# kubernetes-sigs/scheduler-plugins

Hardware: AMD Instinct MI355X
Metric: pod_x_node_filter_score_evals_per_sec (higher is better)
Workload: dtype f32+f64

## Files before the change

### include/spx.h

```cpp
#ifndef SPX_H
#define SPX_H

#include <stdint.h>

#ifdef __cplusplus
extern "C" {
#endif


#define SPX_OK 0
#define SPX_ERR_ARG (-1)
#define SPX_ERR_HIP (-2)
#define SPX_ERR_STATE (-3)
#define SPX_ERR_NOGPU (-4)

#define SPX_PLUGIN_ALLOCATABLE 0
#define SPX_PLUGIN_TLP 1
#define SPX_PLUGIN_LVRB 2
#define SPX_PLUGIN_NRT 3
#define SPX_PLUGIN_NETOVERHEAD 4
#define SPX_PLUGIN_CAPACITY 5
#define SPX_PLUGIN_TOPOSORT 6
#define SPX_PLUGIN_LROC 7
#define SPX_PLUGIN_PEAKS 8
// ... 751 lines not shown
#define SPX_OPT_PEAKS_POD_CLASSES 8
#define SPX_OPT_NRT_LN_LIST_PERMILLE 9
#define SPX_OPT_COMMIT_COOP 10
#define SPX_OPT_NRT_RANK_FILTER 11
#define SPX_OPT_ROW_WORKGROUP 12
#define SPX_OPT_TLP_AMB_TABLE 13
#define SPX_OPT_NRT_PACKED_SCORE 14
#define SPX_OPT_NET_ALLOC_FUSED 15
#define SPX_OPT_NRT_RANK_NARROW 16
#define SPX_OPT_PEAKS_ESTIMATE 17
#define SPX_OPT_NRT_FUSED 18
#define SPX_OPT_NRT_WIDE 19
#define SPX_OPT_ALLOC_TABLE_KEEP 20
#define SPX_OPT_TLP_POD_CLASSES 21
#define SPX_OPT_TLP_CHUNK_SCHED 22
#define SPX_NUM_OPTIONS 23
int spx_set_option(spx_engine* e, int option, int64_t value);
int spx_get_option(const spx_engine* e, int option, int64_t* value);

int spx_nrt_pod_classes(const spx_engine* e, int64_t* n_unique, int64_t* n_copies);
int spx_peaks_pod_classes(const spx_engine* e, int64_t* n_unique, int64_t* n_copies);

int spx_tlp_pod_classes(const spx_engine* e, int64_t* rows_evaluated, int64_t* rows_copied);
int spx_tlp_form(const spx_engine* e);
int spx_tlp_fetch_order(spx_engine* e, int32_t* rows);

int spx_sysched_pod_classes(const spx_engine* e, int64_t* n_unique, int64_t* n_copies);

int spx_load_trimaran(spx_engine* e, const spx_node_objects* nodes, const spx_resource_classes* rc, const spx_pod_objects* pods, const spx_metrics_objects* metrics, const spx_assigned_objects* assigned);
int spx_load_trimaran_pods(spx_engine* e, const spx_pod_objects* pods);
int spx_load_nrt(spx_engine* e, const spx_node_objects* nodes, const spx_nrt_objects* nrt, const spx_resource_classes* rc, const spx_pod_objects* pods, const spx_nrt_params* params);
int spx_last_load_nrt_ms(const spx_engine* e, double* ms6);
int spx_load_network(spx_engine* e, const spx_node_objects* nodes, const spx_pod_objects* pods, const spx_appgroup_objects* appgroups, const spx_nettopo_objects* nettopo);
int spx_load_quota(spx_engine* e, const spx_pod_objects* pods, const spx_resource_classes* rc, const spx_quota_objects* quota);
int spx_load_sysched(spx_engine* e, const spx_sysched_objects* o);
typedef struct spx_profile_objects {
  const spx_node_objects* nodes;
  const spx_resource_classes* rc;
  const spx_pod_objects* pods;
  const spx_metrics_objects* metrics;
// ... 133 lines not shown
```

### scheduler-plugins_amd/csrc/kernels_tlp_order.hip

```cpp
#include <hip/hip_runtime.h>

#include "spx_internal.h"

namespace spx {
namespace {

constexpr int kBlock = 1024;
constexpr int kSlots = 2 * kBlock;
constexpr uint32_t kEmpty = 0xffffffffu;

__device__ __forceinline__ uint32_t order_bin(int64_t v, int32_t amb_size) {
  return (v >= 0 && v < static_cast<int64_t>(amb_size)) ? static_cast<uint32_t>(v) : static_cast<uint32_t>(amb_size);
}

__device__ __forceinline__ void block_count(uint32_t* skey, uint32_t* scnt, bool live, uint32_t bin, uint32_t* slot, uint32_t* rank) {
  for (int s = threadIdx.x; s < kSlots; s += kBlock) skey[s] = kEmpty, scnt[s] = 0u;
  __syncthreads();
  *slot = 0u, *rank = 0u;
  if (live) {
    uint32_t s = (bin * 2654435761u) >> 21;
    for (;;) {
      const uint32_t prev = atomicCAS(skey + s, kEmpty, bin);
      if (prev == kEmpty || prev == bin) break;
      s = (s + 1u) & (kSlots - 1);
// ... 18 lines not shown
__device__ __forceinline__ uint32_t block_sum(uint32_t v, uint32_t* wsum) {
#pragma unroll
  for (int m = 32; m >= 1; m >>= 1) v += static_cast<uint32_t>(__shfl_xor(static_cast<int>(v), m));
  if ((threadIdx.x & 63) == 0) wsum[threadIdx.x >> 6] = v;
  __syncthreads();
  uint32_t total = 0;
#pragma unroll
  for (int w = 0; w < kBlock / 64; ++w) total += wsum[w];
  __syncthreads();
  return total;
}

__global__ __launch_bounds__(kBlock) void k_tlp_order_totals(const uint32_t* hist, int n_bins, uint32_t* totals) {
  __shared__ uint32_t wsum[kBlock / 64];
  const int b = blockIdx.x * kBlock + threadIdx.x;
  const uint32_t total = block_sum(b < n_bins ? hist[b] : 0u, wsum);
  if (threadIdx.x == 0) totals[blockIdx.x] = total;
}

__global__ __launch_bounds__(kBlock) void k_tlp_order_scan(uint32_t* hist, int n_bins, const uint32_t* totals, uint32_t* other_start, uint32_t* evaluated) {
  __shared__ uint32_t wsum[kBlock / 64];
  const int t = threadIdx.x, lane = t & 63, wave = t >> 6;
  uint32_t mine = 0;
  for (int i = t; i < static_cast<int>(blockIdx.x); i += kBlock) mine += totals[i];
  const uint32_t carry = block_sum(mine, wsum);
  const int b = blockIdx.x * kBlock + t;
  const uint32_t c = b < n_bins ? hist[b] : 0u;
  uint32_t x = c;
#pragma unroll
  for (int d = 1; d < 64; d <<= 1) {
    const uint32_t y = static_cast<uint32_t>(__shfl_up(static_cast<int>(x), d));
    if (lane >= d) x += y;
  }
  if (lane == 63) wsum[wave] = x;
  __syncthreads();
  uint32_t before = 0;
#pragma unroll
  for (int w = 0; w < kBlock / 64; ++w) before += w < wave ? wsum[w] : 0u;
  __syncthreads();
  const uint32_t o = carry + before + x - c;
  uint32_t ev = 0;
  if (b < n_bins) {
    hist[b] = o;
    if (b == n_bins - 1) *other_start = o;
    else if (c > 0u) ev = 1u + ((o + c - 1u) >> 6) - (o >> 6);
  }
  ev = block_sum(ev, wsum);
  if (t == 0 && ev != 0u) atomicAdd(evaluated, ev);
}

__global__ __launch_bounds__(kBlock) void k_tlp_order_scatter(const int64_t* pod, int64_t n, int32_t amb_size, uint32_t* cursor, int32_t* order) {
  __shared__ uint32_t skey[kSlots], scnt[kSlots];
  const int64_t r = static_cast<int64_t>(blockIdx.x) * kBlock + threadIdx.x;
  const bool live = r < n;
  uint32_t slot, rank;
  block_count(skey, scnt, live, live ? order_bin(pod[r], amb_size) : 0u, &slot, &rank);
  for (int s = threadIdx.x; s < kSlots; s += kBlock)
    if (skey[s] != kEmpty) scnt[s] = atomicAdd(cursor + skey[s], scnt[s]);
  __syncthreads();
  if (live) {
    const uint64_t pos = static_cast<uint64_t>(scnt[slot]) + rank;
    if (pos < static_cast<uint64_t>(n)) order[pos] = static_cast<int32_t>(r);
  }
}

__global__ __launch_bounds__(256) void k_tlp_order_count_key(const int64_t* pod, int64_t n, int32_t amb_size, const int32_t* order, const uint32_t* other_start,
                                                             uint32_t* evaluated, uint32_t* keys, int64_t n_chunks) {
  const int64_t p = static_cast<int64_t>(blockIdx.x) * blockDim.x + threadIdx.x;
  const uint32_t last = static_cast<uint32_t>(n - 1);
  bool ev = false, outside = false;
  if (p < n) {
    const int64_t v = pod[min(static_cast<uint32_t>(order[p]), last)];
    ev = (p & 63) == 0 || v != pod[min(static_cast<uint32_t>(order[p - 1]), last)];
    outside = order_bin(v, amb_size) == static_cast<uint32_t>(amb_size);
  }
  const unsigned long long m = __ballot(ev), mo = __ballot(ev && p >= static_cast<int64_t>(*other_start)), out = __ballot(outside);
  if ((threadIdx.x & 63) == 0) {
// ... 46 lines not shown
      for (int w = 0; w < kBlock / 64; ++w) add += wcnt[w][t], wcnt[w][t] = 0u;
      base[t] += add;
    }
    __syncthreads();
  }
}

__global__ __launch_bounds__(256) void k_tlp_order_move(int64_t n, const int32_t* sorted, const uint32_t* dest, int64_t n_chunks, int32_t* order) {
  const int64_t p = static_cast<int64_t>(blockIdx.x) * blockDim.x + threadIdx.x;
  if (p >= n) return;
  int64_t chunk = p >> 6;
  if (chunk < n_chunks) chunk = min(static_cast<int64_t>(dest[chunk]), n_chunks - 1);
  order[chunk * 64 + (p & 63)] = sorted[p];
}

}

static size_t scan_blocks(int32_t amb_size) { return (static_cast<size_t>(amb_size) + 1 + kBlock - 1) / kBlock; }
size_t tlp_order_scratch_words(int32_t amb_size, int64_t n_rows) {
  return static_cast<size_t>(amb_size) + 3 + scan_blocks(amb_size) + 2 * static_cast<size_t>(n_rows / 64) + static_cast<size_t>(n_rows);
}
size_t tlp_order_evaluated_word(int32_t amb_size) { return static_cast<size_t>(amb_size) + 2; }

void launch_tlp_order(const int64_t* pod_milli, int64_t n_rows, int32_t amb_size, bool chunk_sched, int32_t* order, uint32_t* scratch, hipStream_t s) {
  const int n_bins = amb_size + 1;
  const unsigned blocks = static_cast<unsigned>((n_rows + kBlock - 1) / kBlock), rows256 = static_cast<unsigned>((n_rows + 255) / 256);
  const unsigned sblocks = static_cast<unsigned>(scan_blocks(amb_size));
  const int64_t n_chunks = n_rows / 64;
  uint32_t* other_start = scratch + n_bins;
  uint32_t* evaluated = other_start + 1;
  uint32_t* totals = evaluated + 1;
  uint32_t* keys = totals + sblocks;
  uint32_t* dest = keys + n_chunks;
  const bool sched = chunk_sched && n_chunks > 1;
  int32_t* sorted = sched ? reinterpret_cast<int32_t*>(dest + n_chunks) : order;
  (void)hipMemsetAsync(scratch, 0, (static_cast<size_t>(n_bins) + 2) * sizeof(uint32_t), s);
  hipLaunchKernelGGL(k_tlp_order_hist, dim3(blocks), dim3(kBlock), 0, s, pod_milli, n_rows, amb_size, scratch);
  hipLaunchKernelGGL(k_tlp_order_totals, dim3(sblocks), dim3(kBlock), 0, s, scratch, n_bins, totals);
  hipLaunchKernelGGL(k_tlp_order_scan, dim3(sblocks), dim3(kBlock), 0, s, scratch, n_bins, totals, other_start, evaluated);
  hipLaunchKernelGGL(k_tlp_order_scatter, dim3(blocks), dim3(kBlock), 0, s, pod_milli, n_rows, amb_size, scratch, sorted);
  hipLaunchKernelGGL(k_tlp_order_count_key, dim3(rows256), dim3(256), 0, s, pod_milli, n_rows, amb_size, sorted, other_start, evaluated, keys, n_chunks);
  if (!sched) return;
  hipLaunchKernelGGL(k_tlp_order_sched, dim3(1), dim3(kBlock), 0, s, keys, n_chunks, dest);
  hipLaunchKernelGGL(k_tlp_order_move, dim3(rows256), dim3(256), 0, s, n_rows, sorted, dest, n_chunks, order);
}

}
```

### scheduler-plugins_amd/csrc/spx_engine.h

```cpp
#pragma once

#include <hip/hip_runtime.h>

#include <algorithm>
#include <chrono>
#include <cmath>
#include <cstdio>
#include <cstdlib>
#include <cstring>
#include <limits>
#include <string>
#include <unordered_map>
#include <vector>

#include <atomic>
#include <mutex>
#include <thread>

#include "spx_internal.h"
#include "../host/lroc_form.hpp"
#include "../host/nrt_streams.hpp"
#include "../host/parallel.hpp"

extern thread_local std::string g_create_error;
// ... 16 lines not shown
  hipStream_t own_stream = nullptr;
  hipStream_t stream = nullptr;
  hipEvent_t ev0 = nullptr, ev1 = nullptr;
  bool hold_ev0 = false;
  bool skip_alloc_masked = false;
  bool alloc_compact = false;
  bool timed = false;
  mutable std::string err;
  mutable std::mutex err_mu;
  std::mutex raw_mu;

  int64_t n_nodes = -1;
  int64_t n_pods = -1;
  int64_t row_stride = 0;

  int64_t option[SPX_NUM_OPTIONS] = {spx::kRowPad, 0, 0, 0, 0, 0, 44, 1, 1, 375, 1, 1, 0, 1, 1, 1, 1, 1, 1, 0, 1, 1, 1};

  int32_t alloc_mode = SPX_MODE_LEAST;
  std::vector<int32_t> alloc_res{SPX_RES_MEMORY, SPX_RES_CPU};
  std::vector<int64_t> alloc_weight{1, 1 << 20};
  spx_tlp_params tlp{40, 1000, 1.5};
  spx_lvrb_params lvrb{1.0, 1.0};
  int64_t plugin_weight[SPX_NUM_PLUGINS] = {1, 1, 1, 1, 1, 1, 1, 1, 1, 1};

  DevBuf d_alloc, d_alloc_w, d_alloc_raw, d_alloc_norm, d_alloc_rel;
  int32_t alloc_n_res = 0;
  bool alloc_ready = false;
  DevBuf d_alloc_prev;
  uint64_t alloc_epoch = 0;
  DevBuf d_cap_cpu, d_tlp_util, d_tlp_missing, d_tlp_valid;
  DevBuf d_lv_acpu, d_lv_amem, d_lv_cavg, d_lv_cstd, d_lv_mavg, d_lv_mstd, d_lv_flags;
  bool tri_nodes = false;
  DevBuf d_tlp_pod, d_lv_rcpu, d_lv_rmem;
  bool tri_pods = false;
  DevBuf d_raw_row;
  DevBuf d_lv_exact;
  DevBuf d_lv_fast, d_tlp_fast;
  DevBuf d_tlp_amb;
  DevBuf d_lv_amb;
  bool lv_amb_built = false;
  int64_t tlp_amb_geom[3] = {0, 0, 0}, lv_amb_geom[3] = {0, 0, 0};
  bool tlp_amb_built = false;
  DevBuf d_tlp_order, d_tlp_order_scratch;
  bool tlp_order_valid = false;
  int64_t tlp_rows_evaluated = 0;
  int tlp_last_form = 0;
  DevBuf d_commit;
  DevBuf d_decide;
  DevBuf d_stats;

  spx_lroc_params lroc{5, 0.5, 0.5};
  DevBuf d_lroc_nreq_c, d_lroc_nreq_m, d_lroc_nlim_c, d_lroc_nlim_m, d_lroc_preq_c, d_lroc_preq_m, d_lroc_plim_c, d_lroc_plim_m, d_lroc_tab, d_lroc_podf;
  bool lroc_nodes = false, lroc_pods = false, lroc_tab_ready = false;
  bool lroc_nodes_exact = false, lroc_pods_exact = false, lv_alloc_exact = false;
  bool lroc_nodes_f32 = false, lroc_pods_f32 = false, lv_alloc_f32 = false;
  int64_t lroc_node_max[4] = {0, 0, 0, 0};
  std::vector<int64_t> h_lroc_pod[4];
  bool lroc_nodes_cover = false, lroc_pods_cover = false;
  int lroc_loop_form = -1;
  bool peaks_loop_row = false;
  int lroc_last_form = -1;
// ... 244 lines not shown
}

int set_pods(spx_engine* e, int64_t p) {
  if (p <= 0) return fail(e, SPX_ERR_ARG, "n_pods must be positive");
  if (e->n_pods != -1 && e->n_pods != p)
    return fail(e, SPX_ERR_STATE, "n_pods differs from tables already uploaded");
  e->n_pods = p;
  return SPX_OK;
}

int tlp_build_order(spx_engine* e) {
  e->tlp_order_valid = false;
  if (e->n_pods <= 0 || e->n_pods > std::numeric_limits<int32_t>::max()) return SPX_OK;
  int rc;
  const size_t words = spx::tlp_order_scratch_words(spx::kTlpAmbSize, e->n_pods);
  if ((rc = ensure(e, e->d_tlp_order, static_cast<size_t>(e->n_pods) * sizeof(int32_t))) || (rc = ensure(e, e->d_tlp_order_scratch, words * sizeof(uint32_t))))
    return rc;
  uint32_t* scratch = static_cast<uint32_t*>(e->d_tlp_order_scratch.p);
  spx::launch_tlp_order(static_cast<const int64_t*>(e->d_tlp_pod.p), e->n_pods, spx::kTlpAmbSize, e->option[SPX_OPT_TLP_CHUNK_SCHED] != 0,
                        static_cast<int32_t*>(e->d_tlp_order.p), scratch, e->stream);
  SPX_HIP(e, hipGetLastError());
  uint32_t evaluated = 0;
  SPX_HIP(e, hipMemcpyAsync(&evaluated, scratch + spx::tlp_order_evaluated_word(spx::kTlpAmbSize), sizeof evaluated, hipMemcpyDeviceToHost, e->stream));
  SPX_HIP(e, hipStreamSynchronize(e->stream));
  e->tlp_rows_evaluated = evaluated;
  e->tlp_order_valid = true;
  return SPX_OK;
}

void alloc_table_dirty(spx_engine* e) { e->alloc_kept = spx_engine::AllocKept{}; }

int ensure_score_table(spx_engine* e, int plugin) {
  DevBuf& b = e->score[plugin];
  if (b.external) {
    if (e->score_rows[plugin] < e->n_pods || e->score_stride[plugin] < e->row_stride)
      return fail(e, SPX_ERR_STATE, "bound score table is smaller than n_pods x row_stride");
    return SPX_OK;
  }
  const size_t had = b.p ? b.bytes : 0;
  int rc = ensure(e, b, static_cast<size_t>(e->n_pods) * static_cast<size_t>(e->row_stride));
// ... 528 lines not shown
```

### scheduler-plugins_amd/csrc/spx_engine.hip

```cpp
#include "spx_engine.h"

thread_local std::string g_create_error;
thread_local std::string tl_err;
thread_local const spx_engine* tl_err_engine = nullptr;

extern "C" {

int spx_abi_version(void) { return 1; }

const char* spx_last_error(const spx_engine* e) {
  if (!e) return g_create_error.c_str();
  if (tl_err_engine != e) {
    std::lock_guard<std::mutex> g(e->err_mu);
    tl_err = e->err;
    tl_err_engine = e;
  }
  return tl_err.c_str();
}

int spx_create(int device_id, spx_engine** out) {
  if (!out) return fail(nullptr, SPX_ERR_ARG, "out is NULL");
  *out = nullptr;
  int count = 0;
  hipError_t st = hipGetDeviceCount(&count);
// ... 16 lines not shown
    delete e;
    return fail(nullptr, SPX_ERR_HIP, msg);
  }
  e->d_stats.bytes = spx::kStatBytes;
  *out = e;
  return SPX_OK;
}

int spx_destroy(spx_engine* e) {
  if (!e) return SPX_OK;
  (void)hipSetDevice(e->device);
  (void)hipStreamSynchronize(e->stream);
  DevBuf* bufs[] = {&e->d_alloc,   &e->d_alloc_w,  &e->d_alloc_raw, &e->d_alloc_norm, &e->d_alloc_rel, &e->d_alloc_prev, &e->d_cap_cpu, &e->d_tlp_util,
                    &e->d_tlp_missing, &e->d_tlp_valid, &e->d_lv_acpu, &e->d_lv_amem, &e->d_lv_cavg, &e->d_lv_cstd,
                    &e->d_lv_mavg, &e->d_lv_mstd,  &e->d_lv_flags,  &e->d_tlp_pod,    &e->d_lv_rcpu, &e->d_lv_rmem,
                    &e->d_raw_row,   &e->d_lv_exact, &e->d_lv_fast, &e->d_tlp_fast, &e->d_tlp_amb, &e->d_tlp_order, &e->d_tlp_order_scratch, &e->d_lv_amb, &e->d_nrt_pk_tab, &e->d_commit, &e->d_nrt_flags, &e->d_nrt_max_numa, &e->d_nrt_nz, &e->d_nrt_zid, &e->d_nrt_zp,
                    &e->d_nrt_avail, &e->d_nrt_cost,  &e->d_nrt_minavg, &e->d_nrt_np,    &e->d_nrt_qos, &e->d_nrt_nn,
                    &e->d_nrt_nctr,  &e->d_nrt_ckind, &e->d_nrt_cpres,  &e->d_nrt_creq,  &e->d_nrt_ppres, &e->d_nrt_preq,
                    &e->d_nrt_frcv, &e->d_nrt_fav,   &e->d_nrt_frc,   &e->d_nrt_fcpu,   &e->d_nrt_frep,  &e->d_nrt_items, &e->d_nrt_perm, &e->d_nrt_ln, &e->d_nrt_fbraw, &e->d_nrt_redo,
                    &e->d_net_region, &e->d_net_zone, &e->d_net_class, &e->d_net_class16, &e->d_net_cls_size, &e->d_net_cls_region, &e->d_net_cls_zone,
                    &e->d_net_rcost, &e->d_net_zcost, &e->d_net_pod_key, &e->d_net_key_flag, &e->d_net_pair_ptr,
                    &e->d_net_pair_node, &e->d_net_pair_max, &e->d_q_pod_ns, &e->d_q_pod_prio, &e->d_q_pod_req, &e->d_q_pod_reqp,
                    &e->d_q_has, &e->d_q_used, &e->d_q_max, &e->d_q_maxp, &e->d_q_other, &e->d_q_otherp, &e->d_q_nom_ptr,
                    &e->d_q_nom_prio, &e->d_q_nom_idx, &e->d_q_nom_req, &e->d_q_nom_reqp, &e->d_q_status, &e->d_ext_status,
                    &e->d_q_usedp, &e->d_q_min, &e->d_q_minp, &e->d_q_agg, &e->d_net_eff_ptr, &e->d_net_eff_key, &e->d_net_eff_cost, &e->d_net_dyn_ptr,
                    &e->d_net_dyn_end, &e->d_net_dyn_node, &e->d_net_dyn_max, &e->d_commit_save, &e->d_row_counter, &e->d_coop_sync, &e->d_coop_node, &e->d_coop_max,
                    &e->d_sort_prio, &e->d_sort_ts, &e->d_sort_group, &e->d_sort_topo, &e->d_sort_scratch,
                    &e->d_best, &e->d_stats, &e->d_decide, &e->d_lroc_nreq_c, &e->d_lroc_nreq_m, &e->d_lroc_nlim_c, &e->d_lroc_nlim_m,
                    &e->d_lroc_preq_c, &e->d_lroc_preq_m, &e->d_lroc_plim_c, &e->d_lroc_plim_m, &e->d_lroc_tab, &e->d_lroc_podf,
                    &e->d_pk_cap, &e->d_pk_util, &e->d_pk_valid, &e->d_pk_k1, &e->d_pk_k2, &e->d_pk_pod, &e->d_pk_min, &e->d_pk_max, &e->d_pk_rowc, &e->d_pk_tab, &e->d_pk_seg, &e->d_pk_segn,
                    &e->d_nrt_uniq, &e->d_nrt_dups, &e->d_pk_uniq, &e->d_pk_dups, &e->d_delta, &e->d_nrt_lnrec, &e->d_net_pair_node2, &e->d_net_pair_max2, &e->d_nrt_rk, &e->d_nrt_rk_off, &e->d_nrt_rk_first, &e->d_nrt_fz, &e->d_nrt_wsort, &e->d_nrt_wrank,
// ... 59 lines not shown
    case SPX_OPT_COMMIT_COOP:
    case SPX_OPT_NRT_RANK_FILTER:
    case SPX_OPT_ROW_WORKGROUP:
    case SPX_OPT_TLP_AMB_TABLE:
    case SPX_OPT_NRT_PACKED_SCORE:
    case SPX_OPT_NET_ALLOC_FUSED:
    case SPX_OPT_NRT_RANK_NARROW:
    case SPX_OPT_NRT_FUSED:
    case SPX_OPT_NRT_WIDE:
    case SPX_OPT_ALLOC_TABLE_KEEP:
    case SPX_OPT_TLP_CHUNK_SCHED:
      if (value != 0 && value != 1) return fail(e, SPX_ERR_ARG, "option takes 0 or 1");
      break;
    case SPX_OPT_TLP_POD_CLASSES:
      if (value < 0 || value > 2) return fail(e, SPX_ERR_ARG, "SPX_OPT_TLP_POD_CLASSES: 0, 1 or 2");
      break;
    case SPX_OPT_NRT_LN_LIST_PERMILLE:
      if (value < 1 || value > 1000) return fail(e, SPX_ERR_ARG, "SPX_OPT_NRT_LN_LIST_PERMILLE: 1..1000");
      break;
    case SPX_OPT_PEAKS_ESTIMATE:
      if (value != 0 && value != 1 && value != 8) return fail(e, SPX_ERR_ARG, "SPX_OPT_PEAKS_ESTIMATE: 0, 1 or 8");
      break;
    case SPX_OPT_PEAKS_TILE:
      if (value != 44 && value != 84 && value != 48 && value != 88) return fail(e, SPX_ERR_ARG, "SPX_OPT_PEAKS_TILE: 44, 84, 48 or 88");
      break;
    default:
      return fail(e, SPX_ERR_ARG, "unknown option");
  }
  e->option[option] = value;
  return SPX_OK;
// ... 532 lines not shown
  if (rows_copied) *rows_copied = e->n_pods - e->tlp_rows_evaluated;
  return SPX_OK;
}

int spx_tlp_form(const spx_engine* e) { return e ? e->tlp_last_form : 0; }

int spx_tlp_fetch_order(spx_engine* e, int32_t* rows) {
  if (!e || !rows) return SPX_ERR_ARG;
  if (!e->tri_pods || !e->tlp_order_valid) return fail(e, SPX_ERR_STATE, "TargetLoadPacking: no row order (no pod batch uploaded, or more than 2^31 - 1 rows)");
  const size_t n = static_cast<size_t>(e->n_pods);
  SPX_HIP(e, hipMemcpyAsync(rows, e->d_tlp_order.p, n * sizeof(int32_t), hipMemcpyDeviceToHost, e->stream));
  SPX_HIP(e, hipStreamSynchronize(e->stream));
  return SPX_OK;
}

int spx_nrt_wide(const spx_engine* e) { return e && e->nrt_wide ? 1 : 0; }

int spx_nrt_long_rows(const spx_engine* e, int64_t* n_out) {
  if (!e || !n_out) return SPX_ERR_ARG;
  *n_out = e->nrt_long_last;
  return SPX_OK;
}

int spx_nrt_packed_score_slots(const spx_engine* e) {
  if (!e) return SPX_ERR_ARG;
  NrtPacked pk;
  if (!nrt_packed_score(e, &pk)) return 0;
  return static_cast<int>(0x1000000u | pk.small_slots | (static_cast<uint32_t>(pk.tab_slot + 1) << 16));
}

// ... 439 lines not shown
namespace {
int decide_profile(spx_engine* e, uint32_t plugin_mask, int64_t row_begin, int64_t row_end) {
  const uint32_t A = 1u << SPX_PLUGIN_ALLOCATABLE, T = 1u << SPX_PLUGIN_TLP;
  const int kExtra[3] = {SPX_PLUGIN_LVRB, SPX_PLUGIN_LROC, SPX_PLUGIN_PEAKS};
  uint32_t extra_mask = 0;
  int64_t w_sum = 0;
  bool w_ok = true;
  for (int p = 0; p < SPX_NUM_PLUGINS; ++p)
    if (plugin_mask & (1u << p)) w_sum += e->plugin_weight[p], w_ok &= e->plugin_weight[p] >= 0;
  for (int x = 0; x < 3; ++x) extra_mask |= plugin_mask & (1u << kExtra[x]);
  const int64_t wa = e->plugin_weight[SPX_PLUGIN_ALLOCATABLE], wt = e->plugin_weight[SPX_PLUGIN_TLP];
  const bool fusable = (plugin_mask & T) && !(plugin_mask & ~(A | T | extra_mask)) && !e->ext_mask && e->tri_nodes && e->tri_pods &&
                       e->tlp.target_utilization >= 1 && e->tlp.target_utilization <= 99 && !(launch_opts(e) & spx::kOptTrimaranExact) &&
                       !e->option[SPX_OPT_DECIDE_UNFUSED] && w_ok && w_sum <= 8000;
  int rc;
  if (!fusable) {
    bool done = false;
    if ((rc = decide_masked(e, plugin_mask, plugin_mask, row_begin, row_end, &done)) || done) return rc;
  }
  if (!fusable) {
    if ((rc = spx_eval(e, plugin_mask, row_begin, row_end))) return rc;
    return spx_eval_best(e, plugin_mask, row_begin, row_end);
  }
  if (e->n_nodes <= 0 || e->n_pods <= 0) return fail(e, SPX_ERR_STATE, "shape unknown");
  if (row_begin < 0 || row_end > e->n_pods || row_begin > row_end) return fail(e, SPX_ERR_ARG, "row range out of bounds");
  const bool use_alloc = plugin_mask & A;
  if (use_alloc && (rc = prepare_alloc(e))) return rc;
  const size_t P = static_cast<size_t>(e->n_pods);
  if ((rc = ensure(e, e->d_best, P * 20))) return rc;
  if ((rc = ensure(e, e->d_tlp_fast, static_cast<size_t>(spx::round_up(e->row_stride, 1024)) * 4 * sizeof(float)))) return rc;
  if ((rc = ensure(e, e->d_decide, spx::decide_scratch_bytes(e->row_stride, row_end - row_begin)))) return rc;
  spx::DecideLaunch d{};
  fill_trimaran(e, d.t);
  d.t.row_begin = row_begin;
  d.t.row_end = row_end;
  d.t.tlp_fast = static_cast<float*>(e->d_tlp_fast.p);
  if (!e->d_tlp_amb.p) e->tlp_amb_built = false;
  if ((rc = ensure(e, e->d_tlp_amb, static_cast<size_t>(spx::kTlpAmbSize) * 4))) return rc;
  d.t.tlp_amb = static_cast<uint32_t*>(e->d_tlp_amb.p);
  d.t.tlp_amb_size = spx::kTlpAmbSize;
  d.t.tlp_amb_built = &e->tlp_amb_built;
  d.t.tlp_amb_geom = e->tlp_amb_geom;
  d.use_alloc = use_alloc;
  d.w_alloc = static_cast<int32_t>(use_alloc ? wa : 0);
  d.w_tlp = static_cast<int32_t>(wt);
  d.scratch = e->d_decide.p;
  d.best_score = static_cast<int64_t*>(e->d_best.p);
  d.best_node = reinterpret_cast<int32_t*>(d.best_score + P);
  d.best_ties = d.best_node + P;
  d.best_feasible = d.best_ties + P;
  SPX_HIP(e, hipEventRecord(e->ev0, e->stream));
  if (extra_mask) {
    e->hold_ev0 = true;
    rc = spx_eval(e, extra_mask, row_begin, row_end);
    e->hold_ev0 = false;
    if (rc) return rc;
    for (int x = 0; x < 3; ++x)
      if (extra_mask & (1u << kExtra[x])) {
        d.w_extra[d.n_extra] = static_cast<int32_t>(e->plugin_weight[kExtra[x]]);
        d.extra[d.n_extra++] = static_cast<const uint8_t*>(e->score[kExtra[x]].p);
      }
  }
  spx::launch_decide_trimaran(d, e->stream);
  SPX_HIP(e, hipGetLastError());
  SPX_HIP(e, hipEventRecord(e->ev1, e->stream));
  e->timed = true;
  e->best_valid = true;
  return SPX_OK;
}
}

extern "C" {

int spx_fetch_best(spx_engine* e, int64_t row_begin, int64_t row_end, int32_t* node_idx, int64_t* weighted_score, int32_t* n_ties,
                   int32_t* n_feasible) {
  if (!e || !node_idx || !weighted_score) return SPX_ERR_ARG;
  if (!e->best_valid) return fail(e, SPX_ERR_STATE, "spx_eval_best has not run since the last spx_eval");
  if (row_begin < 0 || row_end > e->n_pods || row_begin > row_end) return fail(e, SPX_ERR_ARG, "row range out of bounds");
  const size_t n = static_cast<size_t>(row_end - row_begin);
  const size_t P = static_cast<size_t>(e->n_pods);
  if (e->h_best_bytes < P * 20) {
    if (e->h_best) SPX_HIP(e, hipHostFree(e->h_best));
// ... 19 lines not shown
```

### scheduler-plugins_amd/csrc/spx_internal.h

```cpp
#pragma once

#include <hip/hip_runtime.h>
#include <stdint.h>

#include "../../include/spx.h"
#include "nrt_rank_layout.h"

namespace spx {

constexpr int64_t kRowAlign = 16;
constexpr int64_t kRowPad = 128;

inline int64_t round_up(int64_t v, int64_t a) { return (v + a - 1) / a * a; }

#define SPX_RESOLVE_ROWS(a)              \
  do {                                   \
    if ((a).row_ptr) {                   \
      (a).row_begin = *(a).row_ptr;      \
      (a).row_end = (a).row_begin + 1;   \
    }                                    \
  } while (0)

constexpr int kStatSlots = 64;
constexpr int kStatStride = 16;
// ... 26 lines not shown

struct AllocPrepArgs {
  int64_t n_nodes;
  int64_t row_stride;
  int32_t n_res;
  int32_t mode;
  const int64_t* alloc;
  const int64_t* weight;
  int64_t* raw;
  uint8_t* norm;
  uint32_t* rel;
};
void launch_alloc_prepare(const AllocPrepArgs& a, hipStream_t s);

constexpr int64_t kTlpClassMinCopyPct = 47;
constexpr int32_t kTlpAmbSize = 1 << 16;

struct TrimaranArgs {
  uint32_t opts;
  int64_t n_nodes;
  int64_t row_stride;
  int64_t row_begin;
  int64_t row_end;
  const int64_t* row_ptr;
  const uint8_t* alloc_norm;
  const int64_t* cap_cpu_milli;
  const double* tlp_cpu_util;
  const int64_t* tlp_missing_milli;
  const uint8_t* tlp_valid;
  const int64_t* tlp_pod_milli;
// ... 17 lines not shown
  uint32_t* lv_amb;
  int64_t* tlp_amb_geom;
  int64_t* lv_amb_geom;
  bool* lv_amb_built;
  bool* tlp_amb_built;
  const int32_t* tlp_order;
  int* tlp_form;
  unsigned long long* stats;
  uint8_t* out_alloc;
  uint8_t* out_tlp;
  uint8_t* out_lvrb;
};
void launch_trimaran(const TrimaranArgs& a, hipStream_t s);
size_t tlp_order_scratch_words(int32_t amb_size, int64_t n_rows);
size_t tlp_order_evaluated_word(int32_t amb_size);
void launch_tlp_order(const int64_t* pod_milli, int64_t n_rows, int32_t amb_size, bool chunk_sched, int32_t* order, uint32_t* scratch, hipStream_t s);
size_t lvrb_amb_bytes();
struct CommitArgs {
  TrimaranArgs t;
  uint32_t use_mask;
  int64_t w_alloc, w_tlp, w_lvrb;
  const uint8_t* lv_table;
  int64_t* missing;
  int32_t* out_node;
  int64_t* out_score;
  int32_t* out_ties;
};
void launch_commit_trimaran(const CommitArgs& c, hipStream_t s);
struct DecideLaunch {
  TrimaranArgs t;
  bool use_alloc;
// ... 857 lines not shown
```

### scheduler-plugins_amd/engine.py

```python
from __future__ import annotations

import ctypes as C
from typing import Dict, Optional, Sequence

import numpy as np

from ._abi import Table

PLUGINS = {
    "NodeResourcesAllocatable": 0,
    "TargetLoadPacking": 1,
    "LoadVariationRiskBalancing": 2,
    "NodeResourceTopologyMatch": 3,
    "NetworkOverhead": 4,
    "CapacityScheduling": 5,
    "TopologicalSort": 6,
}
ALLOCATABLE, TLP, LVRB, NRT, NETOVERHEAD, CAPACITY, TOPOSORT, LROC, PEAKS, SYSCHED = range(10)
NUM_PLUGINS = 10
COSCHED = 10
COSCHED_ST = {"BACKED_OFF": 1, "FEW_SIBLINGS": 2, "GATED": 3, "RESOURCE_GAP": 4}
PREEMPT_ST = {"CANDIDATE": 0, "NO_VICTIMS": 1, "NOT_FIT": 2, "QUOTA": 3, "ALL_REPRIEVED": 4, "REMOVE_TWICE": 5, "SKIPPED": 6}


# ... 117 lines not shown
        self._ck(self._lib.spx_peaks_pod_classes(self._h, C.byref(u), C.byref(d)))
        return int(u.value), int(d.value)

    def tlp_pod_classes(self):
        u, d = C.c_int64(), C.c_int64()
        self._ck(self._lib.spx_tlp_pod_classes(self._h, C.byref(u), C.byref(d)))
        return int(u.value), int(d.value)

    def tlp_order(self):
        rows = np.zeros(self.n_pods, np.int32)
        self._ck(self._lib.spx_tlp_fetch_order(self._h, rows.ctypes.data_as(C.POINTER(C.c_int32))))
        return rows

    def tlp_form(self) -> int:
        return int(self._lib.spx_tlp_form(self._h))

    def sysched_pod_classes(self):
        u, d = C.c_int64(), C.c_int64()
        self._ck(self._lib.spx_sysched_pod_classes(self._h, C.byref(u), C.byref(d)))
        return int(u.value), int(d.value)

    def force_reference_kernels(self, *plugins: int) -> None:
        self.set_option("REFERENCE_KERNELS", mask_of(*plugins))

    def stats(self, reset: bool = False) -> np.ndarray:
        out = np.zeros(NUM_PLUGINS, np.int64)
        self._ck(self._lib.spx_fetch_stats(self._h, out.ctypes.data_as(C.POINTER(C.c_int64)), 1 if reset else 0))
        return out

    def set_allocatable(self, mode: str = "Least", resources: Optional[Dict[int, int]] = None) -> None:
# ... 1036 lines not shown
```

Measured before the change: 4885 billion.

## Deduplicate pods by CPU request class in fused decide, then expand per row

Extends the TLP ordering pass to assign each pod row a class id, one per distinct in-range CPU milli value, with out-of-range rows each getting their own class. It also records a representative value per class. When enough rows are duplicates, the fused decide kernel runs once per class and a new expand kernel copies the per-class best score, node, ties and feasibility back to every row. This is meant to cut node-by-pod work whenever many pods share the same request. The cost is extra scan and scatter work, more scratch memory, and an added expand launch. Correctness depends on the decide result depending only on the per-pod CPU value.

```diff
diff --git a/include/spx.h b/include/spx.h
--- a/include/spx.h
+++ b/include/spx.h
@@ -789,7 +789,8 @@
 #define SPX_OPT_ALLOC_TABLE_KEEP 20
 #define SPX_OPT_TLP_POD_CLASSES 21
 #define SPX_OPT_TLP_CHUNK_SCHED 22
-#define SPX_NUM_OPTIONS 23
+#define SPX_OPT_DECIDE_POD_CLASSES 23
+#define SPX_NUM_OPTIONS 24
 int spx_set_option(spx_engine* e, int option, int64_t value);
 int spx_get_option(const spx_engine* e, int option, int64_t* value);
 
@@ -799,6 +800,8 @@
 int spx_tlp_pod_classes(const spx_engine* e, int64_t* rows_evaluated, int64_t* rows_copied);
 int spx_tlp_form(const spx_engine* e);
 int spx_tlp_fetch_order(spx_engine* e, int32_t* rows);
+int spx_decide_pod_classes(const spx_engine* e, int64_t* n_classes, int64_t* n_copies);
+int spx_decide_form(const spx_engine* e);
 
 int spx_sysched_pod_classes(const spx_engine* e, int64_t* n_unique, int64_t* n_copies);
 
diff --git a/scheduler-plugins_amd/csrc/kernels_tlp_order.hip b/scheduler-plugins_amd/csrc/kernels_tlp_order.hip
--- a/scheduler-plugins_amd/csrc/kernels_tlp_order.hip
+++ b/scheduler-plugins_amd/csrc/kernels_tlp_order.hip
@@ -56,31 +56,41 @@
 __global__ __launch_bounds__(kBlock) void k_tlp_order_totals(const uint32_t* hist, int n_bins, uint32_t* totals) {
   __shared__ uint32_t wsum[kBlock / 64];
   const int b = blockIdx.x * kBlock + threadIdx.x;
-  const uint32_t total = block_sum(b < n_bins ? hist[b] : 0u, wsum);
-  if (threadIdx.x == 0) totals[blockIdx.x] = total;
-}
-
-__global__ __launch_bounds__(kBlock) void k_tlp_order_scan(uint32_t* hist, int n_bins, const uint32_t* totals, uint32_t* other_start, uint32_t* evaluated) {
-  __shared__ uint32_t wsum[kBlock / 64];
+  const uint32_t c = b < n_bins ? hist[b] : 0u;
+  const uint32_t total = block_sum(c, wsum);
+  const uint32_t taken = block_sum((c > 0u && b < n_bins - 1) ? 1u : 0u, wsum);
+  if (threadIdx.x == 0) totals[blockIdx.x] = total, totals[gridDim.x + blockIdx.x] = taken;
+}
+
+__global__ __launch_bounds__(kBlock) void k_tlp_order_scan(uint32_t* hist, int n_bins, const uint32_t* totals, uint32_t* other_start, uint32_t* evaluated,
+                                                           uint32_t* bin_class, int64_t* class_val, int64_t n_rows, uint32_t* n_classes) {
+  __shared__ uint32_t wsum[kBlock / 64], wsum_k[kBlock / 64];
   const int t = threadIdx.x, lane = t & 63, wave = t >> 6;
-  uint32_t mine = 0;
-  for (int i = t; i < static_cast<int>(blockIdx.x); i += kBlock) mine += totals[i];
-  const uint32_t carry = block_sum(mine, wsum);
+  uint32_t mine = 0, mine_k = 0;
+  for (int i = t; i < static_cast<int>(blockIdx.x); i += kBlock) mine += totals[i], mine_k += totals[gridDim.x + i];
+  const uint32_t carry = block_sum(mine, wsum), carry_k = block_sum(mine_k, wsum);
   const int b = blockIdx.x * kBlock + t;
   const uint32_t c = b < n_bins ? hist[b] : 0u;
-  uint32_t x = c;
+  const uint32_t k = (c > 0u && b < n_bins - 1) ? 1u : 0u;
+  uint32_t x = c, xk = k;
 #pragma unroll
   for (int d = 1; d < 64; d <<= 1) {
-    const uint32_t y = static_cast<uint32_t>(__shfl_up(static_cast<int>(x), d));
-    if (lane >= d) x += y;
-  }
-  if (lane == 63) wsum[wave] = x;
-  __syncthreads();
-  uint32_t before = 0;
-#pragma unroll
-  for (int w = 0; w < kBlock / 64; ++w) before += w < wave ? wsum[w] : 0u;
+    const uint32_t y = static_cast<uint32_t>(__shfl_up(static_cast<int>(x), d)), yk = static_cast<uint32_t>(__shfl_up(static_cast<int>(xk), d));
+    if (lane >= d) x += y, xk += yk;
+  }
+  if (lane == 63) wsum[wave] = x, wsum_k[wave] = xk;
+  __syncthreads();
+  uint32_t before = 0, before_k = 0;
+#pragma unroll
+  for (int w = 0; w < kBlock / 64; ++w) before += w < wave ? wsum[w] : 0u, before_k += w < wave ? wsum_k[w] : 0u;
   __syncthreads();
   const uint32_t o = carry + before + x - c;
+  const uint32_t cls = carry_k + before_k + xk - k;
+  if (b < n_bins) {
+    bin_class[b] = cls;
+    if (k != 0u && static_cast<int64_t>(cls) < n_rows) class_val[cls] = b;
+    if (b == n_bins - 1) *n_classes = cls + c;
+  }
   uint32_t ev = 0;
   if (b < n_bins) {
     hist[b] = o;
@@ -91,18 +101,27 @@
   if (t == 0 && ev != 0u) atomicAdd(evaluated, ev);
 }
 
-__global__ __launch_bounds__(kBlock) void k_tlp_order_scatter(const int64_t* pod, int64_t n, int32_t amb_size, uint32_t* cursor, int32_t* order) {
+__global__ __launch_bounds__(kBlock) void k_tlp_order_scatter(const int64_t* pod, int64_t n, int32_t amb_size, uint32_t* cursor, int32_t* order,
+                                                              const uint32_t* bin_class, const uint32_t* other_start, int64_t* class_val, int32_t* class_of_row) {
   __shared__ uint32_t skey[kSlots], scnt[kSlots];
   const int64_t r = static_cast<int64_t>(blockIdx.x) * kBlock + threadIdx.x;
   const bool live = r < n;
   uint32_t slot, rank;
-  block_count(skey, scnt, live, live ? order_bin(pod[r], amb_size) : 0u, &slot, &rank);
+  const int64_t v = live ? pod[r] : 0;
+  const uint32_t bin = live ? order_bin(v, amb_size) : 0u;
+  block_count(skey, scnt, live, bin, &slot, &rank);
   for (int s = threadIdx.x; s < kSlots; s += kBlock)
     if (skey[s] != kEmpty) scnt[s] = atomicAdd(cursor + skey[s], scnt[s]);
   __syncthreads();
   if (live) {
     const uint64_t pos = static_cast<uint64_t>(scnt[slot]) + rank;
     if (pos < static_cast<uint64_t>(n)) order[pos] = static_cast<int32_t>(r);
+    uint64_t cls = bin_class[bin];
+    if (bin == static_cast<uint32_t>(amb_size)) {
+      cls += pos - *other_start;
+      if (cls < static_cast<uint64_t>(n)) class_val[cls] = v;
+    }
+    class_of_row[r] = static_cast<int32_t>(min(cls, static_cast<uint64_t>(n - 1)));
   }
 }
 
@@ -179,35 +198,60 @@
   order[chunk * 64 + (p & 63)] = sorted[p];
 }
 
+__global__ __launch_bounds__(256) void k_decide_expand(const int32_t* class_of_row, int64_t n_rows, int64_t n_classes, const int64_t* c_score, const int32_t* c_node,
+                                                       const int32_t* c_ties, const int32_t* c_feasible, int64_t* best_score, int32_t* best_node,
+                                                       int32_t* best_ties, int32_t* best_feasible) {
+  const int64_t r = static_cast<int64_t>(blockIdx.x) * blockDim.x + threadIdx.x;
+  if (r >= n_rows) return;
+  const int64_t c = min(static_cast<int64_t>(static_cast<uint32_t>(class_of_row[r])), n_classes - 1);
+  best_score[r] = c_score[c];
+  best_node[r] = c_node[c];
+  best_ties[r] = c_ties[c];
+  best_feasible[r] = c_feasible[c];
+}
+
 }
 
 static size_t scan_blocks(int32_t amb_size) { return (static_cast<size_t>(amb_size) + 1 + kBlock - 1) / kBlock; }
 size_t tlp_order_scratch_words(int32_t amb_size, int64_t n_rows) {
-  return static_cast<size_t>(amb_size) + 3 + scan_blocks(amb_size) + 2 * static_cast<size_t>(n_rows / 64) + static_cast<size_t>(n_rows);
+  return 2 * (static_cast<size_t>(amb_size) + 1) + 3 + 2 * scan_blocks(amb_size) + 2 * static_cast<size_t>(n_rows / 64) + static_cast<size_t>(n_rows);
 }
 size_t tlp_order_evaluated_word(int32_t amb_size) { return static_cast<size_t>(amb_size) + 2; }
 
-void launch_tlp_order(const int64_t* pod_milli, int64_t n_rows, int32_t amb_size, bool chunk_sched, int32_t* order, uint32_t* scratch, hipStream_t s) {
+void launch_tlp_order(const int64_t* pod_milli, int64_t n_rows, int32_t amb_size, bool chunk_sched, int32_t* order, int64_t* class_val, int32_t* class_of_row,
+                      uint32_t* scratch, hipStream_t s) {
   const int n_bins = amb_size + 1;
   const unsigned blocks = static_cast<unsigned>((n_rows + kBlock - 1) / kBlock), rows256 = static_cast<unsigned>((n_rows + 255) / 256);
   const unsigned sblocks = static_cast<unsigned>(scan_blocks(amb_size));
   const int64_t n_chunks = n_rows / 64;
   uint32_t* other_start = scratch + n_bins;
   uint32_t* evaluated = other_start + 1;
-  uint32_t* totals = evaluated + 1;
-  uint32_t* keys = totals + sblocks;
+  uint32_t* n_classes = evaluated + 1;
+  uint32_t* totals = n_classes + 1;
+  uint32_t* bin_class = totals + 2 * sblocks;
+  uint32_t* keys = bin_class + n_bins;
   uint32_t* dest = keys + n_chunks;
   const bool sched = chunk_sched && n_chunks > 1;
   int32_t* sorted = sched ? reinterpret_cast<int32_t*>(dest + n_chunks) : order;
   (void)hipMemsetAsync(scratch, 0, (static_cast<size_t>(n_bins) + 2) * sizeof(uint32_t), s);
   hipLaunchKernelGGL(k_tlp_order_hist, dim3(blocks), dim3(kBlock), 0, s, pod_milli, n_rows, amb_size, scratch);
   hipLaunchKernelGGL(k_tlp_order_totals, dim3(sblocks), dim3(kBlock), 0, s, scratch, n_bins, totals);
-  hipLaunchKernelGGL(k_tlp_order_scan, dim3(sblocks), dim3(kBlock), 0, s, scratch, n_bins, totals, other_start, evaluated);
-  hipLaunchKernelGGL(k_tlp_order_scatter, dim3(blocks), dim3(kBlock), 0, s, pod_milli, n_rows, amb_size, scratch, sorted);
+  hipLaunchKernelGGL(k_tlp_order_scan, dim3(sblocks), dim3(kBlock), 0, s, scratch, n_bins, totals, other_start, evaluated, bin_class, class_val, n_rows, n_classes);
+  hipLaunchKernelGGL(k_tlp_order_scatter, dim3(blocks), dim3(kBlock), 0, s, pod_milli, n_rows, amb_size, scratch, sorted, bin_class, other_start, class_val, class_of_row);
   hipLaunchKernelGGL(k_tlp_order_count_key, dim3(rows256), dim3(256), 0, s, pod_milli, n_rows, amb_size, sorted, other_start, evaluated, keys, n_chunks);
   if (!sched) return;
   hipLaunchKernelGGL(k_tlp_order_sched, dim3(1), dim3(kBlock), 0, s, keys, n_chunks, dest);
   hipLaunchKernelGGL(k_tlp_order_move, dim3(rows256), dim3(256), 0, s, n_rows, sorted, dest, n_chunks, order);
 }
 
-}
+void launch_decide_expand(const int32_t* class_of_row, int64_t n_rows, int64_t n_classes, const void* class_best, void* best, hipStream_t s) {
+  if (n_rows <= 0 || n_classes <= 0) return;
+  const int64_t* cs = static_cast<const int64_t*>(class_best);
+  const int32_t* cn = reinterpret_cast<const int32_t*>(cs + n_classes);
+  int64_t* bs = static_cast<int64_t*>(best);
+  int32_t* bn = reinterpret_cast<int32_t*>(bs + n_rows);
+  hipLaunchKernelGGL(k_decide_expand, dim3(static_cast<unsigned>((n_rows + 255) / 256)), dim3(256), 0, s, class_of_row, n_rows, n_classes, cs, cn, cn + n_classes,
+                     cn + 2 * n_classes, bs, bn, bn + n_rows, bn + 2 * n_rows);
+}
+
+}
diff --git a/scheduler-plugins_amd/csrc/spx_engine.h b/scheduler-plugins_amd/csrc/spx_engine.h
--- a/scheduler-plugins_amd/csrc/spx_engine.h
+++ b/scheduler-plugins_amd/csrc/spx_engine.h
@@ -54,7 +54,7 @@
   int64_t n_pods = -1;
   int64_t row_stride = 0;
 
-  int64_t option[SPX_NUM_OPTIONS] = {spx::kRowPad, 0, 0, 0, 0, 0, 44, 1, 1, 375, 1, 1, 0, 1, 1, 1, 1, 1, 1, 0, 1, 1, 1};
+  int64_t option[SPX_NUM_OPTIONS] = {spx::kRowPad, 0, 0, 0, 0, 0, 44, 1, 1, 375, 1, 1, 0, 1, 1, 1, 1, 1, 1, 0, 1, 1, 1, 1};
 
   int32_t alloc_mode = SPX_MODE_LEAST;
   std::vector<int32_t> alloc_res{SPX_RES_MEMORY, SPX_RES_CPU};
@@ -85,6 +85,9 @@
   bool tlp_order_valid = false;
   int64_t tlp_rows_evaluated = 0;
   int tlp_last_form = 0;
+  DevBuf d_tlp_class_val, d_tlp_class_of_row, d_decide_cls;
+  int64_t tlp_n_classes = 0;
+  int decide_last_form = 0;
   DevBuf d_commit;
   DevBuf d_decide;
   DevBuf d_stats;
@@ -359,16 +362,20 @@
   if (e->n_pods <= 0 || e->n_pods > std::numeric_limits<int32_t>::max()) return SPX_OK;
   int rc;
   const size_t words = spx::tlp_order_scratch_words(spx::kTlpAmbSize, e->n_pods);
-  if ((rc = ensure(e, e->d_tlp_order, static_cast<size_t>(e->n_pods) * sizeof(int32_t))) || (rc = ensure(e, e->d_tlp_order_scratch, words * sizeof(uint32_t))))
+  if ((rc = ensure(e, e->d_tlp_order, static_cast<size_t>(e->n_pods) * sizeof(int32_t))) || (rc = ensure(e, e->d_tlp_order_scratch, words * sizeof(uint32_t))) ||
+      (rc = ensure(e, e->d_tlp_class_val, static_cast<size_t>(e->n_pods) * sizeof(int64_t))) ||
+      (rc = ensure(e, e->d_tlp_class_of_row, static_cast<size_t>(e->n_pods) * sizeof(int32_t))))
     return rc;
   uint32_t* scratch = static_cast<uint32_t*>(e->d_tlp_order_scratch.p);
   spx::launch_tlp_order(static_cast<const int64_t*>(e->d_tlp_pod.p), e->n_pods, spx::kTlpAmbSize, e->option[SPX_OPT_TLP_CHUNK_SCHED] != 0,
-                        static_cast<int32_t*>(e->d_tlp_order.p), scratch, e->stream);
+                        static_cast<int32_t*>(e->d_tlp_order.p), static_cast<int64_t*>(e->d_tlp_class_val.p), static_cast<int32_t*>(e->d_tlp_class_of_row.p),
+                        scratch, e->stream);
   SPX_HIP(e, hipGetLastError());
-  uint32_t evaluated = 0;
-  SPX_HIP(e, hipMemcpyAsync(&evaluated, scratch + spx::tlp_order_evaluated_word(spx::kTlpAmbSize), sizeof evaluated, hipMemcpyDeviceToHost, e->stream));
+  uint32_t back[2] = {0, 0};
+  SPX_HIP(e, hipMemcpyAsync(back, scratch + spx::tlp_order_evaluated_word(spx::kTlpAmbSize), sizeof back, hipMemcpyDeviceToHost, e->stream));
   SPX_HIP(e, hipStreamSynchronize(e->stream));
-  e->tlp_rows_evaluated = evaluated;
+  e->tlp_rows_evaluated = back[0];
+  e->tlp_n_classes = std::min<int64_t>(std::max<int64_t>(back[1], 1), e->n_pods);
   e->tlp_order_valid = true;
   return SPX_OK;
 }
diff --git a/scheduler-plugins_amd/csrc/spx_engine.hip b/scheduler-plugins_amd/csrc/spx_engine.hip
--- a/scheduler-plugins_amd/csrc/spx_engine.hip
+++ b/scheduler-plugins_amd/csrc/spx_engine.hip
@@ -54,7 +54,7 @@
   DevBuf* bufs[] = {&e->d_alloc,   &e->d_alloc_w,  &e->d_alloc_raw, &e->d_alloc_norm, &e->d_alloc_rel, &e->d_alloc_prev, &e->d_cap_cpu, &e->d_tlp_util,
                     &e->d_tlp_missing, &e->d_tlp_valid, &e->d_lv_acpu, &e->d_lv_amem, &e->d_lv_cavg, &e->d_lv_cstd,
                     &e->d_lv_mavg, &e->d_lv_mstd,  &e->d_lv_flags,  &e->d_tlp_pod,    &e->d_lv_rcpu, &e->d_lv_rmem,
-                    &e->d_raw_row,   &e->d_lv_exact, &e->d_lv_fast, &e->d_tlp_fast, &e->d_tlp_amb, &e->d_tlp_order, &e->d_tlp_order_scratch, &e->d_lv_amb, &e->d_nrt_pk_tab, &e->d_commit, &e->d_nrt_flags, &e->d_nrt_max_numa, &e->d_nrt_nz, &e->d_nrt_zid, &e->d_nrt_zp,
+                    &e->d_raw_row,   &e->d_lv_exact, &e->d_lv_fast, &e->d_tlp_fast, &e->d_tlp_amb, &e->d_tlp_order, &e->d_tlp_order_scratch, &e->d_tlp_class_val, &e->d_tlp_class_of_row, &e->d_decide_cls, &e->d_lv_amb, &e->d_nrt_pk_tab, &e->d_commit, &e->d_nrt_flags, &e->d_nrt_max_numa, &e->d_nrt_nz, &e->d_nrt_zid, &e->d_nrt_zp,
                     &e->d_nrt_avail, &e->d_nrt_cost,  &e->d_nrt_minavg, &e->d_nrt_np,    &e->d_nrt_qos, &e->d_nrt_nn,
                     &e->d_nrt_nctr,  &e->d_nrt_ckind, &e->d_nrt_cpres,  &e->d_nrt_creq,  &e->d_nrt_ppres, &e->d_nrt_preq,
                     &e->d_nrt_frcv, &e->d_nrt_fav,   &e->d_nrt_frc,   &e->d_nrt_fcpu,   &e->d_nrt_frep,  &e->d_nrt_items, &e->d_nrt_perm, &e->d_nrt_ln, &e->d_nrt_fbraw, &e->d_nrt_redo,
@@ -144,6 +144,9 @@
       break;
     case SPX_OPT_TLP_POD_CLASSES:
       if (value < 0 || value > 2) return fail(e, SPX_ERR_ARG, "SPX_OPT_TLP_POD_CLASSES: 0, 1 or 2");
+      break;
+    case SPX_OPT_DECIDE_POD_CLASSES:
+      if (value < 0 || value > 2) return fail(e, SPX_ERR_ARG, "SPX_OPT_DECIDE_POD_CLASSES: 0, 1 or 2");
       break;
     case SPX_OPT_NRT_LN_LIST_PERMILLE:
       if (value < 1 || value > 1000) return fail(e, SPX_ERR_ARG, "SPX_OPT_NRT_LN_LIST_PERMILLE: 1..1000");
@@ -706,6 +709,16 @@
   return SPX_OK;
 }
 
+int spx_decide_pod_classes(const spx_engine* e, int64_t* n_classes, int64_t* n_copies) {
+  if (!e) return SPX_ERR_ARG;
+  if (!e->tri_pods || !e->tlp_order_valid) return fail(e, SPX_ERR_STATE, "spx_decide: no pod classes (no pod batch uploaded, or more than 2^31 - 1 rows)");
+  if (n_classes) *n_classes = e->tlp_n_classes;
+  if (n_copies) *n_copies = e->n_pods - e->tlp_n_classes;
+  return SPX_OK;
+}
+
+int spx_decide_form(const spx_engine* e) { return e ? e->decide_last_form : 0; }
+
 int spx_nrt_wide(const spx_engine* e) { return e && e->nrt_wide ? 1 : 0; }
 
 int spx_nrt_long_rows(const spx_engine* e, int64_t* n_out) {
@@ -1175,6 +1188,7 @@
                        e->tlp.target_utilization >= 1 && e->tlp.target_utilization <= 99 && !(launch_opts(e) & spx::kOptTrimaranExact) &&
                        !e->option[SPX_OPT_DECIDE_UNFUSED] && w_ok && w_sum <= 8000;
   int rc;
+  e->decide_last_form = 0;
   if (!fusable) {
     bool done = false;
     if ((rc = decide_masked(e, plugin_mask, plugin_mask, row_begin, row_end, &done)) || done) return rc;
@@ -1190,11 +1204,20 @@
   const size_t P = static_cast<size_t>(e->n_pods);
   if ((rc = ensure(e, e->d_best, P * 20))) return rc;
   if ((rc = ensure(e, e->d_tlp_fast, static_cast<size_t>(spx::round_up(e->row_stride, 1024)) * 4 * sizeof(float)))) return rc;
-  if ((rc = ensure(e, e->d_decide, spx::decide_scratch_bytes(e->row_stride, row_end - row_begin)))) return rc;
+  bool cls = false;
+  const int64_t cls_opt = e->option[SPX_OPT_DECIDE_POD_CLASSES];
+  if (cls_opt && !extra_mask && e->tlp_order_valid && row_begin == 0 && row_end == e->n_pods && !e->row_indirect && e->tlp_n_classes > 0) {
+    const int64_t copies = e->n_pods - e->tlp_n_classes;
+    cls = cls_opt == 2 ? copies > 0 : copies * 100 >= spx::kDecideClassMinCopyPct * e->n_pods;
+  }
+  const int64_t C = cls ? e->tlp_n_classes : 0;
+  if ((rc = ensure(e, e->d_decide, spx::decide_scratch_bytes(e->row_stride, cls ? C : row_end - row_begin)))) return rc;
+  if (cls && (rc = ensure(e, e->d_decide_cls, static_cast<size_t>(C) * 20))) return rc;
   spx::DecideLaunch d{};
   fill_trimaran(e, d.t);
   d.t.row_begin = row_begin;
-  d.t.row_end = row_end;
+  d.t.row_end = cls ? C : row_end;
+  if (cls) d.t.tlp_pod_milli = static_cast<const int64_t*>(e->d_tlp_class_val.p);
   d.t.tlp_fast = static_cast<float*>(e->d_tlp_fast.p);
   if (!e->d_tlp_amb.p) e->tlp_amb_built = false;
   if ((rc = ensure(e, e->d_tlp_amb, static_cast<size_t>(spx::kTlpAmbSize) * 4))) return rc;
@@ -1202,6 +1225,7 @@
   d.t.tlp_amb_size = spx::kTlpAmbSize;
   d.t.tlp_amb_built = &e->tlp_amb_built;
   d.t.tlp_amb_geom = e->tlp_amb_geom;
+  if (cls && C < 256) d.t.tlp_amb_built = nullptr;
   d.use_alloc = use_alloc;
   d.w_alloc = static_cast<int32_t>(use_alloc ? wa : 0);
   d.w_tlp = static_cast<int32_t>(wt);
@@ -1210,6 +1234,12 @@
   d.best_node = reinterpret_cast<int32_t*>(d.best_score + P);
   d.best_ties = d.best_node + P;
   d.best_feasible = d.best_ties + P;
+  if (cls) {
+    d.best_score = static_cast<int64_t*>(e->d_decide_cls.p);
+    d.best_node = reinterpret_cast<int32_t*>(d.best_score + C);
+    d.best_ties = d.best_node + C;
+    d.best_feasible = d.best_ties + C;
+  }
   SPX_HIP(e, hipEventRecord(e->ev0, e->stream));
   if (extra_mask) {
     e->hold_ev0 = true;
@@ -1223,10 +1253,12 @@
       }
   }
   spx::launch_decide_trimaran(d, e->stream);
+  if (cls) spx::launch_decide_expand(static_cast<const int32_t*>(e->d_tlp_class_of_row.p), e->n_pods, C, e->d_decide_cls.p, e->d_best.p, e->stream);
   SPX_HIP(e, hipGetLastError());
   SPX_HIP(e, hipEventRecord(e->ev1, e->stream));
   e->timed = true;
   e->best_valid = true;
+  e->decide_last_form = cls ? 2 : 1;
   return SPX_OK;
 }
 }
diff --git a/scheduler-plugins_amd/csrc/spx_internal.h b/scheduler-plugins_amd/csrc/spx_internal.h
--- a/scheduler-plugins_amd/csrc/spx_internal.h
+++ b/scheduler-plugins_amd/csrc/spx_internal.h
@@ -64,6 +64,7 @@
 void launch_alloc_prepare(const AllocPrepArgs& a, hipStream_t s);
 
 constexpr int64_t kTlpClassMinCopyPct = 47;
+constexpr int64_t kDecideClassMinCopyPct = 12;
 constexpr int32_t kTlpAmbSize = 1 << 16;
 
 struct TrimaranArgs {
@@ -111,7 +112,9 @@
 void launch_trimaran(const TrimaranArgs& a, hipStream_t s);
 size_t tlp_order_scratch_words(int32_t amb_size, int64_t n_rows);
 size_t tlp_order_evaluated_word(int32_t amb_size);
-void launch_tlp_order(const int64_t* pod_milli, int64_t n_rows, int32_t amb_size, bool chunk_sched, int32_t* order, uint32_t* scratch, hipStream_t s);
+void launch_tlp_order(const int64_t* pod_milli, int64_t n_rows, int32_t amb_size, bool chunk_sched, int32_t* order, int64_t* class_val, int32_t* class_of_row,
+                      uint32_t* scratch, hipStream_t s);
+void launch_decide_expand(const int32_t* class_of_row, int64_t n_rows, int64_t n_classes, const void* class_best, void* best, hipStream_t s);
 size_t lvrb_amb_bytes();
 struct CommitArgs {
   TrimaranArgs t;
diff --git a/scheduler-plugins_amd/engine.py b/scheduler-plugins_amd/engine.py
--- a/scheduler-plugins_amd/engine.py
+++ b/scheduler-plugins_amd/engine.py
@@ -155,6 +155,14 @@
 
     def tlp_form(self) -> int:
         return int(self._lib.spx_tlp_form(self._h))
+
+    def decide_pod_classes(self):
+        u, d = C.c_int64(), C.c_int64()
+        self._ck(self._lib.spx_decide_pod_classes(self._h, C.byref(u), C.byref(d)))
+        return int(u.value), int(d.value)
+
+    def decide_form(self) -> int:
+        return int(self._lib.spx_decide_form(self._h))
 
     def sysched_pod_classes(self):
         u, d = C.c_int64(), C.c_int64()
```

Result: slower. 4836 billion (-1.0%).
